# pkorus/neural-imaging

Measured on AMD Instinct MI355X. Metric: patches/s (fwd+bwd) ISP->JPEG->FAN @256^2, higher is better.
Workload: dtype bf16; 1 GPU; c4 = train_manipulation UNet->[native,sharpen:1,resample:50,gaussian:0.83,jpeg:80]->dJPEG(QF80,soft)->FAN, ds none, trainable nip+fan, lambda_nip 0.1; raw_patch=128, batch_per_gpu=64, global_batch=64, parallelism=dp1, world_size=1, hip_graph=False

## Files before the change

### include/nimg.h

```cpp
#ifndef NIMG_H
#define NIMG_H

#include <stddef.h>
#include <stdint.h>

#ifdef __cplusplus
extern "C" {
#endif

#define NIMG_OK 0
#define NIMG_ERR_ARG (-1)
#define NIMG_ERR_LAUNCH (-2)
#define NIMG_ERR_WORKSPACE (-3)

#define NIMG_BF16_IN 1
#define NIMG_BF16_OUT 2
#define NIMG_BF16_MASK 4
#define NIMG_BF16_DZ 8
#define NIMG_D2S_OUT 16
#define NIMG_MASK_CONV 128
#define NIMG_COPY_LRELU 64
#define NIMG_S2D_OUT 32
#define NIMG_UNPOOL_OUT 512
#define NIMG_D2S_CONVT 1024
// ... 232 lines not shown
int nimg_latent_fwd(const float* z, const float* scale, const float* codebook, int codebook_size, float v,
                    float gamma, int soft_codebook, float* latent, float* entropy, long count, long count_global,
                    void* workspace, size_t workspace_bytes, int finalize, void* stream);
int nimg_latent_entropy_finalize(int codebook_size, long count_global, float* entropy, void* workspace, void* stream);
int nimg_latent_bwd(const float* z, const float* scale, const float* latent, const float* dlatent,
                    float entropy_coef, const float* codebook, int codebook_size, float v, float gamma,
                    int soft_codebook, float* dz, float* dscale, int accumulate_dscale, long count, void* workspace,
                    size_t workspace_bytes, void* stream);
size_t nimg_l2_loss_workspace_bytes(void);
int nimg_l2_loss(const float* target, const float* y, float* loss, float* grad_y, long count, float grad_scale,
                 int accumulate, void* workspace, size_t workspace_bytes, void* stream);

size_t nimg_conv_weights_bf16_bytes(int ks_h, int ks_w, int cin, int cout, int mode);
int nimg_conv_weights_bf16(const float* w, void* wb, int ks_h, int ks_w, int cin, int cout, int mode, void* stream);
int nimg_conv2d_wgrad_pooled_bf16(const float* in, int cin, const float* g, const unsigned char* idx, int cout,
                                  float* dw, float* db, int n, int h, int wd, int ks, int accumulate, void* workspace,
                                  size_t workspace_bytes, void* stream);
int nimg_conv2d_dgrad_fewin_pooled_bf16(const float* g, const unsigned char* idx, const float* w, float* out, int ci,
                                        int cz, int n, int h, int wd, int ks, void* stream);
int nimg_conv2d_fwd_bf16_ex(const float* in1, int c1, const float* in2, int c2, const void* wb, const float* bias,
                            float* out1, int o1, float* out2, int o2, const float* act_mask, int n, int h, int wd,
                            int ks, int stride, int pad_t, int pad_l, int pad_mode, int hout, int wout, int act,
                            float alpha, int flags, void* stream);
int nimg_conv2d_wgrad_bf16_ex(const float* in1, int c1, const float* in2, int c2, const float* dz, int cout, float* dw,
                              float* db, int n, int h, int wd, int ks, int stride, int pad_t, int pad_l, int pad_mode,
                              int hout, int wout, int accumulate, void* workspace, size_t workspace_bytes, int flags,
                              void* stream);
int nimg_conv2d_pool_fwd_bf16_ex(const float* in, int cin, const float* w, const void* wb, const float* bias,
                                 float* pool_out, unsigned char* pool_idx, int cout, int n, int h, int wd, int ks,
                                 int act, float alpha, int flags, void* stream);
int nimg_conv2d_fwd_pool_also_bf16(const float* in, int cin, const void* wb, const float* bias, float* out, float* pool_out,
                                   unsigned char* pool_idx, int cout, int n, int h, int wd, int act, float alpha, void* stream);
#define NIMG_ROWS_F32_OUT 1
int nimg_conv3_rows_bf16(const void* in1, int c1, const void* in2, int c2, const void* wb, const float* bias, const void* mask,
                         void* out, void* out2, void* pool_out, int n, int h, int wd, int cout, int act, float alpha, int flags,
                         void* stream);
int nimg_conv3_rows_d2s_bf16(const void* in, int c1, const void* wb, const float* bias, float* y, int n, int h, int wd, void* stream);
int nimg_conv3_rows_c4_bf16(const float* in, const float* w, const float* bias, void* out, int n, int h, int wd, int act, float alpha,
                            void* stream);

int nimg_conv2d_dgrad_unpool_out_bf16(const float* dz, int c1, const void* wb, const float* act, const float* skip, float* out,
                                      int cout, int n, int h, int wd, int apply_mask, float alpha, void* stream);
int nimg_conv2d_wgrad_pooled_bf16_ex(const float* in, int cin, const float* g, const unsigned char* idx, int cout,
                                     float* dw, float* db, int n, int h, int wd, int ks, int accumulate, void* workspace,
                                     size_t workspace_bytes, int flags, void* stream);
int nimg_conv2d_dgrad_fewin_pooled_bf16_ex(const float* g, const unsigned char* idx, const float* w, float* out, int ci,
                                           int cz, int n, int h, int wd, int ks, int flags, void* stream);
int nimg_maxpool2_unpool_ex(const float* dp, const unsigned char* idx, const float* pooled, float* dz, int n, int ho,
                            int wo, int c, int apply_lrelu_mask, float alpha, int flags, void* stream);
int nimg_convt2x2_fwd_bf16(const float* x, const void* wb, const float* bias, float* y, int n, int h, int wd, int cin,
                           int cout, void* stream);
int nimg_convt2x2_fwd_bf16_ex(const float* x, const void* wb, const float* bias, float* y, int n, int h, int wd, int cin,
                              int cout, int flags, void* stream);
int nimg_conv_weights_bf16_batch(const void* table, int n_entries, void* stream);
int nimg_conv2d_fwd_bf16(const float* in1, int c1, const float* in2, int c2, const void* wb, const float* bias,
                         float* out1, int o1, float* out2, int o2, const float* act_mask, int n, int h, int wd,
                         int ks, int stride, int pad_t, int pad_l, int pad_mode, int hout, int wout, int act,
                         float alpha, void* stream);
size_t nimg_conv2d_wgrad_bf16_workspace_bytes(int cin, int cout, int ks_h, int ks_w, int n, int hout, int wout);
int nimg_conv2d_wgrad_bf16(const float* in1, int c1, const float* in2, int c2, const float* dz, int cout, float* dw,
                           float* db, int n, int h, int wd, int ks, int stride, int pad_t, int pad_l, int pad_mode,
                           int hout, int wout, int accumulate, void* workspace, size_t workspace_bytes, void* stream);

int nimg_conv2d_fwd_smallc_bf16(const float* in, int cin, const float* w, const float* bias, float* out, int cout,
                                int n, int h, int wd, int ks, int pad_mode, int act, float alpha, void* stream);
int nimg_conv2d_fwd_smallc_bf16_ex(const float* in, int cin, const float* w, const float* bias, float* out, int cout,
                                   int n, int h, int wd, int ks, int pad_mode, int act, float alpha, int flags, void* stream);
int nimg_conv2d_dgrad_fewin_bf16(const float* dz, const float* w, float* out, int ci, int cz, int n, int h, int wd,
                                 int ks, void* stream);

int nimg_awgn_fwd(const float* x, const float* noise, float* y, uint8_t* mask, long count, float strength,
                  void* stream);
int nimg_awgn_bwd(const float* x, const float* noise, const float* dy, const uint8_t* mask, float* dx, long count,
                  float strength, void* stream);
int nimg_gamma_fwd(const float* x, float* y, long count, float gamma, void* stream);
int nimg_gamma_bwd(const float* x, const float* dy, float* dx, long count, float gamma, void* stream);
int nimg_median_fwd(const float* x, float* y, uint8_t* sel, int n, int h, int w, int kernel, void* stream);
int nimg_median_bwd(const float* dy, const uint8_t* sel, float* dx, int n, int h, int w, int kernel, void* stream);

#define NIMG_L3IC_E_READ 1
#define NIMG_L3IC_E_LANES 2
#define NIMG_L3IC_E_RANGE 4
#define NIMG_L3IC_E_SYMBOL 8
#define NIMG_L3IC_E_FREQ 16
#define NIMG_L3IC_E_VARINT 32
#define NIMG_L3IC_E_ODD 64
#define NIMG_L3IC_E_UNUSED 128
#define NIMG_L3IC_E_STATE 256
#define NIMG_L3IC_E_RLE 512
size_t nimg_l3ic_workspace_bytes(int n_streams, int n_sym);
int nimg_l3ic_quantise(const float* z, const float* codebook, int codebook_size, uint8_t* idx, int* err, int n, int h,
                       int w, int c, void* stream);
int nimg_l3ic_encode(const uint8_t* idx, int n_streams, int n_sym, uint8_t* out, uint32_t* lengths, uint32_t* hist,
                     uint32_t* freq, void* workspace, size_t workspace_bytes, void* stream);
int nimg_l3ic_decode(const uint8_t* data, const uint32_t* offsets, const uint32_t* lengths, const float* codebook,
                     int codebook_size, float* z, uint32_t* err, int n, int h, int w, int c, void* stream);

size_t nimg_jpeg_workspace_bytes(int n, int h, int w, int hs, int vs);
int nimg_jpeg_transform(const void* x, int is_u8, int n, int h, int w, int hs, int vs, int quality, int16_t* coef, void* workspace,
                        size_t workspace_bytes, void* stream);
int nimg_jpeg_encode(const int16_t* coef, int n, int h, int w, int hs, int vs, uint8_t* out, size_t out_capacity, uint32_t* lengths,
                     void* workspace, size_t workspace_bytes, void* stream);
int nimg_jpeg_reconstruct(const int16_t* coef, int n, int h, int w, int hs, int vs, int quality, float* y, void* workspace,
                          size_t workspace_bytes, void* stream);
int nimg_jpeg_transform_items(const void* x, int is_u8, int n_src, int h, int w, int hs, int vs, const uint8_t* quality, int n_items,
                              int16_t* coef, int* err, void* workspace, size_t workspace_bytes, void* stream);
// ... 65 lines not shown
```

### neural-imaging_amd/_lib.py

```python
import ctypes
import os
from ctypes import c_float, c_int, c_long, c_size_t, c_void_p

_HERE = os.path.dirname(os.path.abspath(__file__))
LIB_PATH = os.environ.get('NIMG_LIBPATH') or os.path.join(_HERE, 'libnimg.so')

P = c_void_p

PROTOTYPES = {
    'nimg_abi_version': (c_int, []),
    'nimg_djpeg_fwd': (c_int, [P, P, P, P, P, P, c_int, c_int, c_int, c_int, P]),
    'nimg_djpeg_bwd': (c_int, [P, P, P, P, P, c_int, c_int, c_int, c_int, P]),
    'nimg_djpeg_dq_workspace_bytes': (c_size_t, [c_int, c_int, c_int]),
    'nimg_djpeg_bwd_dq': (c_int, [P, P, P, P, P, P, c_int, c_int, c_int, c_int, c_int, P, c_size_t, P]),
    'nimg_djpeg_sub_workspace_bytes': (c_size_t, [c_int, c_int, c_int, c_int, c_int, c_int]),
    'nimg_djpeg_sub_fwd': (c_int, [P, P, P, P, P, P, c_int, c_int, c_int, c_int, c_int, c_int, P, c_size_t, P]),
    'nimg_djpeg_sub_bwd': (c_int, [P, P, P, P, P, P, c_int, c_int, c_int, c_int, c_int, c_int, c_int, P, c_size_t, P]),
    'nimg_djpeg_entropy_workspace_bytes': (c_size_t, [c_int, c_int, c_int]),
    'nimg_djpeg_entropy_fwd': (c_int, [P, P, c_int, c_int, c_int, c_int, P, P, c_size_t, P]),
    'nimg_djpeg_entropy_bwd': (c_int, [P, P, c_int, c_int, c_int, c_int, c_float, P, c_int, P, c_int, P, c_size_t, P]),
    'nimg_jpeg_qtable': (c_int, [c_int, c_int, P]),
    'nimg_conv2d_fwd': (c_int, [P, c_int, P, c_int, P, P, P, c_int, P, c_int, P, c_int, c_int, c_int, c_int, c_int,
                                c_int, c_int, c_int, c_int, c_int, c_int, c_float, P]),
    'nimg_conv_flip_weights': (c_int, [P, P, c_int, c_int, c_int, c_int, P]),
# ... 94 lines not shown
    'nimg_isp_residual_workspace_bytes': (c_long, []),
    'nimg_isp_residual_bwd': (c_int, [P, P, P, P, P, P, c_long, c_int, P]),
    'nimg_activation_fwd': (c_int, [P, P, c_long, c_int, c_float, P]),
    'nimg_activation_bwd': (c_int, [P, P, P, c_long, c_int, c_float, P]),
    'nimg_sigmoid_fwd': (c_int, [P, P, c_long, P]),
    'nimg_sigmoid_bwd': (c_int, [P, P, P, c_long, P]),
    'nimg_gamma_ste_fwd': (c_int, [P, P, c_long, c_float, c_float, c_float, P]),
    'nimg_gamma_ste_bwd': (c_int, [P, P, P, c_long, c_float, c_float, c_float, P]),
    'nimg_mae255_workspace_bytes': (c_size_t, []),
    'nimg_mae255': (c_int, [P, P, P, P, c_long, c_float, c_int, P, c_size_t, P]),
    'nimg_ssim_loss_workspace_bytes': (c_size_t, [c_int, c_int, c_int, c_int, c_int]),
    'nimg_ssim_loss': (c_int, [P, P, P, P, c_int, c_int, c_int, c_int, c_float, P, c_float, c_int, P, c_size_t, P]),
    'nimg_patch_stats': (c_int, [P, c_int, c_int, c_int, P, P, c_int, c_int, c_int, P, P, P]),
    'nimg_patch_select': (c_int, [P, P, P, P, c_int, c_int, c_int, c_int, P, P, P]),
    'nimg_patch_gather': (c_int, [P, P, c_int, c_int, c_int, P, P, c_int, c_int, P, P, P]),
    'nimg_mask_scale': (c_int, [P, P, P, c_long, c_float, P]),
    'nimg_conv5_dgrad_sparse_image_bytes': (c_size_t, [c_int, c_int]),
    'nimg_conv5_dgrad_sparse_weights': (c_int, [P, P, c_int, c_int, P]),
    'nimg_conv5_dgrad_sparse': (c_int, [P, P, c_int, P, P, c_int, P, c_int, c_int, c_int, c_float, c_int, P]),
    'nimg_conv2d_fwd_bf16_res': (c_int, [P, c_int, P, P, P, c_int, P, P, P, c_int, c_int, c_int, c_int, c_int, c_int, c_int, c_int, c_int,
                                 c_int, c_int, c_float, c_int, P]),
    'nimg_conv2d_fwd_bf16_unpool': (c_int, [P, P, c_int, P, P, P, c_int, P, c_int, c_int, c_int, c_int, c_int, c_int, c_int,
                                            c_int, c_int, c_float, c_int, P]),
    'nimg_conv2d_wgrad_bf16_unpool': (c_int, [P, c_int, P, P, c_int, P, P, c_int, c_int, c_int, c_int, c_int, P, c_size_t, P]),
    'nimg_cconv3': (c_int, [P, P, P, P, c_int, c_int, c_int, c_int, P]),
    'nimg_conv5c3_bf16': (c_int, [P, P, P, c_int, c_int, c_int, P]),
    'nimg_cconv3_dgrad_border': (c_int, [P, P, P, c_int, c_int, c_int, P]),
    'nimg_cconv3_dgrad_border_strips': (c_int, [P, P, P, c_int, c_int, c_int, P]),
    'nimg_conv1_pool_fwd_c4': (c_int, [P, P, P, P, P, c_int, c_int, c_int, c_float, c_int, P]),
    'nimg_conv1_wgrad_c4_workspace_bytes': (c_size_t, []),
    'nimg_conv1_wgrad_c4': (c_int, [P, P, P, P, P, c_int, c_int, c_int, c_int, c_int, P, c_size_t, P]),
    'nimg_conv1_dgrad_pooled': (c_int, [P, P, P, P, c_int, c_int, c_int, c_int, P]),
    'nimg_confusion_accumulate': (c_int, [P, P, P, P, c_int, c_int, P]),
    'nimg_ssim_planes_workspace_bytes': (c_size_t, [c_int, c_int]),
    'nimg_ssim_planes': (c_int, [P, P, c_int, c_int, c_int, c_int, c_float, P, P, P, P, c_int, P, c_size_t, P]),
    'nimg_msssim_combine': (c_int, [P, P, c_int, c_int, P, P, P]),
    'nimg_ssim_maps_grad': (c_int, [P, P, P, P, P, c_int, c_int, c_int, c_int, P, c_float, c_int, P]),
    'nimg_pad2d': (c_int, [P, P, c_int, c_int, c_int, c_int, c_int, c_int, P]),
    'nimg_conv2d_fwd_bf16_ex': (c_int, [P, c_int, P, c_int, P, P, P, c_int, P, c_int, P, c_int, c_int, c_int, c_int, c_int,
                                        c_int, c_int, c_int, c_int, c_int, c_int, c_float, c_int, P]),
    'nimg_conv2d_wgrad_bf16_ex': (c_int, [P, c_int, P, c_int, P, c_int, P, P, c_int, c_int, c_int, c_int, c_int, c_int,
                                          c_int, c_int, c_int, c_int, c_int, P, c_size_t, c_int, P]),
    'nimg_conv2d_pool_fwd_bf16_ex': (c_int, [P, c_int, P, P, P, P, P, c_int, c_int, c_int, c_int, c_int, c_int, c_float,
                                             c_int, P]),
    'nimg_conv2d_dgrad_unpool_out_bf16': (c_int, [P, c_int, P, P, P, P, c_int, c_int, c_int, c_int, c_int, c_float, P]),
    'nimg_conv2d_fwd_pool_also_bf16': (c_int, [P, c_int, P, P, P, P, P, c_int, c_int, c_int, c_int, c_int, c_float, P]),
    'nimg_conv2d_wgrad_pooled_bf16_ex': (c_int, [P, c_int, P, P, c_int, P, P, c_int, c_int, c_int, c_int, c_int, P,
                                                 c_size_t, c_int, P]),
    'nimg_conv2d_dgrad_fewin_pooled_bf16_ex': (c_int, [P, P, P, P, c_int, c_int, c_int, c_int, c_int, c_int, c_int, P]),
    'nimg_maxpool2_unpool_ex': (c_int, [P, P, P, P, c_int, c_int, c_int, c_int, c_int, c_float, c_int, P]),
    'nimg_conv_weights_bf16_batch': (c_int, [P, c_int, P]),
    'nimg_convt2x2_fwd_bf16': (c_int, [P, P, P, P, c_int, c_int, c_int, c_int, c_int, P]),
    'nimg_convt2x2_fwd_bf16_ex': (c_int, [P, P, P, P, c_int, c_int, c_int, c_int, c_int, c_int, P]),
    'nimg_conv2d_fwd_smallc_bf16': (c_int, [P, c_int, P, P, P, c_int, c_int, c_int, c_int, c_int, c_int, c_int,
                                            c_float, P]),
    'nimg_conv2d_fwd_smallc_bf16_ex': (c_int, [P, c_int, P, P, P, c_int, c_int, c_int, c_int, c_int, c_int, c_int,
                                               c_float, c_int, P]),
    'nimg_conv2d_dgrad_fewin_bf16': (c_int, [P, P, P, c_int, c_int, c_int, c_int, c_int, c_int, P]),
    'nimg_awgn_fwd': (c_int, [P, P, P, P, c_long, c_float, P]),
    'nimg_awgn_bwd': (c_int, [P, P, P, P, P, c_long, c_float, P]),
    'nimg_gamma_fwd': (c_int, [P, P, c_long, c_float, P]),
    'nimg_gamma_bwd': (c_int, [P, P, P, c_long, c_float, P]),
    'nimg_median_fwd': (c_int, [P, P, P, c_int, c_int, c_int, c_int, P]),
    'nimg_median_bwd': (c_int, [P, P, P, c_int, c_int, c_int, c_int, P]),
    'nimg_sparse_axis_apply': (c_int, [P, P, P, P, P, c_int, c_int, c_int, c_int, c_int, c_int, P]),
    'nimg_l3ic_workspace_bytes': (c_size_t, [c_int, c_int]),
    'nimg_l3ic_quantise': (c_int, [P, P, c_int, P, P, c_int, c_int, c_int, c_int, P]),
    'nimg_l3ic_encode': (c_int, [P, c_int, c_int, P, P, P, P, P, c_size_t, P]),
    'nimg_l3ic_decode': (c_int, [P, P, P, P, c_int, P, P, c_int, c_int, c_int, c_int, P]),
    'nimg_jpeg_workspace_bytes': (c_size_t, [c_int, c_int, c_int, c_int, c_int]),
    'nimg_jpeg_transform': (c_int, [P, c_int, c_int, c_int, c_int, c_int, c_int, c_int, P, P, c_size_t, P]),
    'nimg_jpeg_encode': (c_int, [P, c_int, c_int, c_int, c_int, c_int, P, c_size_t, P, P, c_size_t, P]),
    'nimg_jpeg_reconstruct': (c_int, [P, c_int, c_int, c_int, c_int, c_int, c_int, P, P, c_size_t, P]),
    'nimg_jpeg_transform_items': (c_int, [P, c_int, c_int, c_int, c_int, c_int, c_int, P, c_int, P, P, P, c_size_t, P]),
    'nimg_jpeg_reconstruct_items': (c_int, [P, c_int, c_int, c_int, c_int, c_int, P, P, P, P, c_size_t, P]),
    'nimg_jpeg_decode_workspace_bytes': (c_size_t, [c_int, c_int, c_int, c_int, c_int, c_size_t, c_int]),
    'nimg_jpeg_decode': (c_int, [P, P, P, c_int, c_int, c_int, c_int, c_int, c_int, P, P, P, P, c_size_t, P]),
    'nimg_jpeg_reconstruct_tables': (c_int, [P, c_int, c_int, c_int, c_int, c_int, P, P, c_int, P, c_size_t, P]),
    'nimg_jpeg_histogram': (c_int, [P, c_int, c_int, c_int, c_int, c_int, P, P]),
    'nimg_jpeg_optimal_tables': (c_int, [P, c_int, P, P, P]),
    'nimg_jpeg_encode_tables_workspace_bytes': (c_size_t, [c_int, c_int, c_int, c_int, c_int]),
    'nimg_jpeg_encode_tables': (c_int, [P, c_int, c_int, c_int, c_int, c_int, P, P, c_size_t, P, P, P, c_size_t, P]),
    'nimg_jpeg_transform_tables': (c_int, [P, c_int, c_int, c_int, c_int, c_int, c_int, P, c_int, P, P, P, c_size_t, P]),
    'nimg_jpeg_tables_from_float': (c_int, [P, c_int, c_int, P, P, P]),
    'nimg_jpeg_encode_restart_workspace_bytes': (c_size_t, [c_int, c_int, c_int, c_int, c_int, c_int]),
    'nimg_jpeg_encode_restart': (c_int, [P, c_int, c_int, c_int, c_int, c_int, c_int, P, c_size_t, P, P, c_size_t, P]),
    'nimg_jpeg_histogram_restart': (c_int, [P, c_int, c_int, c_int, c_int, c_int, c_int, P, P]),
    'nimg_jpeg_encode_tables_restart_workspace_bytes': (c_size_t, [c_int, c_int, c_int, c_int, c_int, c_int]),
    'nimg_jpeg_encode_tables_restart': (c_int, [P, c_int, c_int, c_int, c_int, c_int, c_int, P, P, c_size_t, P, P, P, c_size_t, P]),
    'nimg_jpeg_decode_restart_workspace_bytes': (c_size_t, [c_int, c_int, c_int, c_int, c_int, c_int, c_size_t, c_int]),
    'nimg_jpeg_decode_restart': (c_int, [P, P, P, c_int, c_int, c_int, c_int, c_int, c_int, c_int, P, P, P, P, c_size_t, P]),
    'nimg_jpeg_decode_progressive_workspace_bytes': (c_size_t, [c_int, c_int, c_int, c_int, c_int, c_int, c_int, c_size_t, c_int]),
    'nimg_jpeg_decode_progressive': (c_int, [P, P, P, c_int, P, c_int, c_int, c_int, c_int, c_int, c_int, c_int, P, P, P, P, c_size_t, P]),
    'nimg_jpeg_progressive_workspace_bytes': (c_size_t, [c_int, c_int, c_int, c_int, c_int, c_int]),
    'nimg_jpeg_progressive_histogram': (c_int, [P, c_int, c_int, c_int, c_int, c_int, c_int, P, P]),
    'nimg_jpeg_encode_progressive': (c_int, [P, c_int, c_int, c_int, c_int, c_int, c_int, P, P, c_size_t, P, P, P, c_size_t, P]),
    'nimg_msssim_workspace_bytes': (c_size_t, [c_int, c_int, c_int, c_int]),
    'nimg_msssim': (c_int, [P, P, c_int, c_int, c_int, c_int, c_float, P, P, P, c_size_t, P]),
    'nimg_conv1_pool_fwd_c4_sign': (c_int, [P, P, P, P, P, P, c_int, c_int, c_int, c_float, c_int, P]),
    'nimg_conv2d_pool_sign_ok': (c_int, [c_int, c_int, c_int, c_int, c_int, c_int, c_int]),
    'nimg_conv2d_pool_fwd_bf16_sign': (c_int, [P, c_int, P, P, P, P, P, P, c_int, c_int, c_int, c_int, c_int, c_int, c_float,
                                               c_int, P]),
    'nimg_conv2d_fwd_bf16_unpool_sign': (c_int, [P, P, c_int, P, P, P, c_int, P, P, c_int, c_int, c_int, c_int, c_int, c_int, c_int,
                                                 c_int, c_int, c_float, c_int, P]),
}

# ... 37 lines not shown
```

### neural-imaging_amd/models/layers.py

```python
import numpy as np
import torch

from .. import ops
from ..helpers import kernels as hk


FUSED_ACTIVATIONS = (None, 'leaky_relu')


def act_forward(y, activation):
    if isinstance(y, tuple):
        raise RuntimeError('a bf16 copy cannot be combined with activation {}'.format(activation))
    return ops.activation(y, activation, out=y)


class Conv2D(object):

    def __init__(self, name, ks, cin, cout, activation=None, stride=1, cin2=0, mask_activation='leaky_relu'):
        self.name, self.ks, self.cin, self.cin2, self.cout = name, ks, cin, cin2, cout
        self.activation, self.stride = activation, stride
        self.mask_activation = mask_activation

    def specs(self):
        return [(self.name + '/kernel', (self.ks, self.ks, self.cin + self.cin2, self.cout)),
# ... 72 lines not shown
        return ops.conv2d_dgrad(dz, store.p[self.name + '/kernel'], in_hw, stride=self.stride, act_mask=act_mask,
                                out=out, out2=out2, out_bf16=out_bf16, residual=residual, bf16_copy=bf16_copy,
                                s2d_out=s2d_out)


class Conv5x5Stride2Image(Conv2D):

    def s2d_ok(self, x):
        return ops.s2d_conv_ok(self.ks, self.stride, x.shape[1], x.shape[2], self.cin) and self.cin2 == 0 and 4 * self.cin <= 16

    def forward_image(self, store, x, a, b, s2d_out=False):
        if not self.s2d_ok(x):
            if s2d_out:
                raise RuntimeError('s2d_out needs the space-to-depth form of the layer')
            x0 = ops.affine(x, a, b)
            return self.forward(store, x0), x0
        xs = ops.s2d2_affine(x, a, b, cp=16)
        w3 = ops.s2d_conv_weights(store.p[self.name + '/kernel'], cp=16)
        fused = self.activation in FUSED_ACTIVATIONS
        y = ops.conv2d(xs, w3, store.p[self.name + '/bias'], act=self.activation if fused else None, s2d_out=s2d_out,
                       out_bf16=s2d_out)
        return (y if fused else act_forward(y, self.activation)), xs

    def backward_params_image(self, store, ctx, dz):
        if ctx.dtype != torch.bfloat16:
            return self.backward_params(store, ctx, dz)
        with ops.side_stream(ctx, dz, key=store.g[self.name + '/kernel'].data_ptr()):
            dw3 = ops.conv2d_wgrad(ctx, dz, 3, db=store.g[self.name + '/bias'])
            ops.s2d_conv_weights_bwd(dw3, store.g[self.name + '/kernel'])

    def backward_input_image(self, store, dz, in_hw, a):
        return ops.conv2d_dgrad_strided2(dz, store.p[self.name + '/kernel'], in_hw, scale=a)


class Conv2DTranspose2x2(object):

    def __init__(self, name, cin, cout):
        self.name, self.cin, self.cout = name, cin, cout

    def specs(self):
        return [(self.name + '/kernel', (2, 2, self.cout, self.cin)), (self.name + '/bias', (self.cout,))]

    def init(self, store, gen):
        from .tfmodel import glorot_uniform_
        k = torch.empty((2, 2, self.cout, self.cin), dtype=torch.float32)
        glorot_uniform_(k, self.cin * 4, self.cout * 4, gen)
        store.p[self.name + '/kernel'].copy_(k)
        store.p[self.name + '/bias'].zero_()

    def forward(self, store, x, out_bf16=False):
        return ops.convt2x2(x, store.p[self.name + '/kernel'], store.p[self.name + '/bias'], out_bf16=out_bf16)

    def backward_params(self, store, x, dy):
        ops.convt2x2_wgrad(x, dy, dw=store.g[self.name + '/kernel'], side=True)
        ops.bias_grad(dy, db=store.g[self.name + '/bias'], side=True)

    def backward_input(self, store, dy, act_mask=None, out_bf16=False, mask_activation='leaky_relu'):
        if act_mask is not None and mask_activation not in FUSED_ACTIVATIONS:
            d = ops.convt2x2_dgrad(dy, store.p[self.name + '/kernel'])
            return ops.activation_bwd(d, act_mask, mask_activation, out=d)
        return ops.convt2x2_dgrad(dy, store.p[self.name + '/kernel'], act_mask=act_mask, out_bf16=out_bf16)


class ConstrainedConv2D(object):

    def __init__(self, name='constrained', filter_strength=100.0):
        self.name, self.strength = name, float(filter_strength)

    def specs(self):
        return [(self.name + '/kernel', (5, 5, 3, 3))]

    def init(self, store, gen=None):
        store.p[self.name + '/kernel'].copy_(torch.from_numpy(hk.residual_init_filter().astype(np.float32)))
        if hasattr(store, 'register_constrained'):
            store.register_constrained(self.name + '/kernel', self.strength)

    _flip = (None, None)

    def forward(self, store, x, c4_only=False):
        cc = getattr(store, 'constrained', None)
        if ops.ADAM_IMAGES and ops.ADAM_CCONV and ops.COMPUTE == 'bf16' and cc is not None and \
                cc['kernel'] is store.p[self.name + '/kernel'] and cc['strength'] == self.strength:
            nf, flip = store.constrained_filter()
            self._flip = (nf, flip)
        else:
            nf = ops.constrained_kernel(store.p[self.name + '/kernel'], self.strength)
            self._flip = (None, None)
        y, c4 = ops.cconv3(x, nf, pad_mode=1, want_f32=not c4_only, want_c4=c4_only)
        return (c4 if c4_only else y), nf

    def backward_params(self, store, x, dy):
        with ops.side_stream(x, dy, key=store.g[self.name + '/kernel'].data_ptr()):
            dnf = ops.conv2d_wgrad(x, dy, 5, pads=(2, 2), pad_mode=1)
            ops.constrained_kernel_bwd(store.p[self.name + '/kernel'], dnf, store.g[self.name + '/kernel'], self.strength)

    def backward_input(self, nf, dy):
        n, h, w, _ = dy.shape
        if h < 4 or w < 4:
            dpad = ops.conv2d(dy, ops.flip_weights(nf), None, pads=(4, 4), out_hw=(h + 4, w + 4))
            return ops.fold_pad(dpad, 2, 1)
        return ops.cconv3_dgrad(dy, nf, nf_flip=self._flip[1] if nf is self._flip[0] else None)
```

### neural-imaging_amd/ops.py

```python
import math
import os

import numpy as np
import torch

from . import _lib

LRELU_ALPHA = 0.2

COMPUTE = 'f32'


STORE_BF16 = True


COMPUTE_EPOCH = 0


def set_compute(mode):
    global COMPUTE, COMPUTE_EPOCH
    if mode not in ('f32', 'bf16'):
        raise ValueError('compute mode must be f32 or bf16')
    if mode != COMPUTE:
        COMPUTE_EPOCH += 1
# ... 778 lines not shown
        return dw
    if _is_bf16(x) or _is_bf16(dz):
        raise RuntimeError('bf16-stored tensor reached a float32 weight-gradient path')
    need = _lib.load().nimg_conv2d_wgrad_workspace_bytes(c1 + c2, cout, ks, ks, n, ho, wo)
    ws = _ws_current(x.device).get(need, x.device)
    _lib.call('nimg_conv2d_wgrad', _p(x), c1, _p(x2), c2, _p(dz), cout, _p(dw), _p(db), n, h, wd, ks, stride, pt, pl,
              pad_mode, ho, wo, 1 if accumulate else 0, _p(ws), ws.numel(), _stream())
    return dw


def _flush_chain_here(k):
    entry = _CHAIN.pop(k, None)
    if entry is not None:
        _lib.call('nimg_reduce_slabs_batch', entry, 1, _stream())


def _wgrad_carried(k, carrier, device, need, flags, *operands):
    import ctypes
    if carrier == 'defer':
        st = _defer_state(k)
        if st['n'] == st['cap']:
            _flush_deferred(k, on_its_stream=False)
        entry = ctypes.byref(st['buf'], st['n'] * st['nb'])
    else:
        entry = (ctypes.c_char * int(_lib.load().nimg_reduce_entry_bytes()))()
    ws = _SIDE['ws'][k].claim(need, device)
    name, pre = ('nimg_conv2d_wgrad_bf16_chained', (_CHAIN.get(k),)) if carrier == 'chain' else ('nimg_conv2d_wgrad_bf16_deferred', ())
    _lib.call(name, *operands, _p(ws), ws.numel(), flags, *pre, entry, _stream())
    if carrier == 'defer':
        st['n'] += 1
    elif carrier == 'chain':
        _CHAIN[k] = entry
    else:
        _reduce_behind(k, entry, device)


def bias_grad(dz, db=None, accumulate=False, side=False):
    if side and _SIDE['enabled'] and db is not None:
        with _on_side_stream(dz, key=db.data_ptr()):
            return bias_grad(dz, db=db, accumulate=accumulate, side=False)
    _f32(db)
    _fb(dz)
    cout = dz.shape[-1]
    npix = dz.numel() // cout
    if db is None:
        db = torch.empty((cout,), dtype=torch.float32, device=dz.device)
    need = _lib.load().nimg_bias_grad_workspace_bytes(npix, cout)
    ws = _ws_current(dz.device).get(need, dz.device)
    _lib.call('nimg_bias_grad_ex', _p(dz), _p(db), npix, cout, 1 if accumulate else 0, _p(ws), ws.numel(),
              BF16_DZ if _is_bf16(dz) else 0, _stream())
    return db


def convt2x2(x, w, bias, out_bf16=False):
    _f32(w, bias)
    _fb(x)
    n, h, wd, cin = x.shape
    cout = w.shape[2]
    y = torch.empty((n, 2 * h, 2 * wd, cout), dtype=torch.bfloat16 if out_bf16 else torch.float32, device=x.device)
    if COMPUTE == 'bf16' and cin % 8 == 0 and cout >= 8:
        wb = weights_bf16(w, 1)
        _lib.call('nimg_convt2x2_fwd_bf16_ex', _p(x), _p(wb), _p(bias), _p(y), n, h, wd, cin, cout,
                  (BF16_IN if _is_bf16(x) else 0) | (BF16_OUT if out_bf16 else 0), _stream())
        return y
    if _is_bf16(x) or out_bf16:
        raise RuntimeError('bf16-stored tensor reached a float32 transposed-convolution path')
    _lib.call('nimg_convt2x2_fwd', _p(x), _p(w), _p(bias), _p(y), n, h, wd, cin, cout, _stream())
    return y


def convt2x2_dgrad(dy, w, act_mask=None, out_bf16=False):
    n, h2, w2, _ = dy.shape
    return conv2d(dy, w, None, stride=2, pads=(0, 0), out_hw=(h2 // 2, w2 // 2), act_mask=act_mask, out_bf16=out_bf16)


def convt2x2_wgrad(x, dy, dw=None, side=False):
    return conv2d_wgrad(dy, x, 2, stride=2, pads=(0, 0), dw=dw, side=side)


def maxpool2(x):
    _fb(x)
    n, h, w, c = x.shape
    y = torch.empty((n, h // 2, w // 2, c), dtype=x.dtype, device=x.device)
    if _is_bf16(x):
        _lib.call('nimg_maxpool2_fwd_bf16', _p(x), _p(y), n, h, w, c, _stream())
        return y
    _lib.call('nimg_maxpool2_fwd', _p(x), _p(y), n, h, w, c, _stream())
    return y


def maxpool2_bwd(dp, yact, add=None, apply_mask=True, out=None, alpha=None):
    a = LRELU_ALPHA if alpha is None else float(alpha)
    _fb(dp, yact, add, out)
    n, h, w, c = yact.shape
    dz = torch.empty_like(yact) if out is None else out
    if _is_bf16(yact):
        if any(t is not None and not _is_bf16(t) for t in (dp, add, dz)):
            raise RuntimeError('maxpool2_bwd on a bf16-stored activation needs bf16-stored gradients')
        _lib.call('nimg_maxpool2_bwd_bf16', _p(dp), _p(yact), _p(add), _p(dz), n, h, w, c, 1 if apply_mask else 0,
                  a, _stream())
        return dz
    _f32(dp, add, dz)
    _lib.call('nimg_maxpool2_bwd', _p(dp), _p(yact), _p(add), _p(dz), n, h, w, c, 1 if apply_mask else 0,
              a, _stream())
    return dz


ACT_SIGN = _os.environ.get('NIMG_NO_ACT_SIGN') is None


def conv2d_pool_sign_ok(x, w, out_bf16=True):
    n, h, wd, cin = x.shape
    return ACT_SIGN and COMPUTE == 'bf16' and _is_bf16(x) and out_bf16 and _lib.load().nimg_conv2d_pool_sign_ok(
        cin, w.shape[3], n, h, wd, w.shape[0], BF16_IN | BF16_OUT) == 1


def conv2d_pool(x, w, bias=None, act='leaky_relu', want_idx=True, out_bf16=False, want_sign=False):
    _f32(w, bias)
    _fb(x)
    n, h, wd, cin = x.shape
    ks, cout = w.shape[0], w.shape[3]
    if w.shape[2] != cin or (h & 1) or (wd & 1) or (cout & 3) or ks not in (3, 5):
        raise ValueError('conv2d_pool: unsupported shape')
    bf16_path = COMPUTE == 'bf16' and (cin in (3, 4) or cin % 8 == 0)
    if (out_bf16 or _is_bf16(x)) and not bf16_path:
        raise RuntimeError('bf16 storage needs the throughput-mode convolution path')
    pooled = torch.empty((n, h // 2, wd // 2, cout), dtype=torch.bfloat16 if out_bf16 else torch.float32, device=x.device)
    idx = torch.empty((n, h // 2, wd // 2, cout), dtype=torch.uint8, device=x.device) if want_idx else None
    a = 1 if act == 'leaky_relu' else 0
    if bf16_path:
# ... 1537 lines not shown
```

Before: 8190 patches/s.

## Add dedicated MFMA GEMM kernels for transposed 2x2 conv fwd, dgrad and fused wgrad+bias

Result: no change. 8214 patches/s, median of 6 (+0.3%).

```diff
diff --git a/include/nimg.h b/include/nimg.h
--- a/include/nimg.h
+++ b/include/nimg.h
@@ -308,6 +308,14 @@
                            int cout, void* stream);
 int nimg_convt2x2_fwd_bf16_ex(const float* x, const void* wb, const float* bias, float* y, int n, int h, int wd, int cin,
                               int cout, int flags, void* stream);
+int nimg_convt2x2_gemm_ok(int pass, int n, int h, int wd, int cin, int cout, int flags);
+int nimg_convt2x2_gemm_fwd(const void* x, const void* wb, const float* bias, void* y, int n, int h, int wd, int cin, int cout,
+                           int flags, void* stream);
+int nimg_convt2x2_gemm_dgrad(const void* dy, const void* wb, const void* mask, void* dx, int n, int h, int wd, int cin, int cout,
+                             float alpha, int flags, void* stream);
+size_t nimg_convt2x2_gemm_wgrad_workspace_bytes(int n, int h, int wd, int cin, int cout);
+int nimg_convt2x2_gemm_wgrad_bias(const void* x, const void* dy, float* dw, float* db, int n, int h, int wd, int cin, int cout,
+                                  void* workspace, size_t workspace_bytes, int flags, void* stream);
 int nimg_conv_weights_bf16_batch(const void* table, int n_entries, void* stream);
 int nimg_conv2d_fwd_bf16(const float* in1, int c1, const float* in2, int c2, const void* wb, const float* bias,
                          float* out1, int o1, float* out2, int o2, const float* act_mask, int n, int h, int wd,
diff --git a/neural-imaging_amd/_lib.py b/neural-imaging_amd/_lib.py
--- a/neural-imaging_amd/_lib.py
+++ b/neural-imaging_amd/_lib.py
@@ -170,6 +170,11 @@
     'nimg_conv_weights_bf16_batch': (c_int, [P, c_int, P]),
     'nimg_convt2x2_fwd_bf16': (c_int, [P, P, P, P, c_int, c_int, c_int, c_int, c_int, P]),
     'nimg_convt2x2_fwd_bf16_ex': (c_int, [P, P, P, P, c_int, c_int, c_int, c_int, c_int, c_int, P]),
+    'nimg_convt2x2_gemm_ok': (c_int, [c_int, c_int, c_int, c_int, c_int, c_int, c_int]),
+    'nimg_convt2x2_gemm_fwd': (c_int, [P, P, P, P, c_int, c_int, c_int, c_int, c_int, c_int, P]),
+    'nimg_convt2x2_gemm_dgrad': (c_int, [P, P, P, P, c_int, c_int, c_int, c_int, c_int, c_float, c_int, P]),
+    'nimg_convt2x2_gemm_wgrad_workspace_bytes': (c_size_t, [c_int, c_int, c_int, c_int, c_int]),
+    'nimg_convt2x2_gemm_wgrad_bias': (c_int, [P, P, P, P, c_int, c_int, c_int, c_int, c_int, P, c_size_t, c_int, P]),
     'nimg_conv2d_fwd_smallc_bf16': (c_int, [P, c_int, P, P, P, c_int, c_int, c_int, c_int, c_int, c_int, c_int,
                                             c_float, P]),
     'nimg_conv2d_fwd_smallc_bf16_ex': (c_int, [P, c_int, P, P, P, c_int, c_int, c_int, c_int, c_int, c_int, c_int,
diff --git a/neural-imaging_amd/csrc/convt2x2.hip b/neural-imaging_amd/csrc/convt2x2.hip
--- /dev/null
+++ b/neural-imaging_amd/csrc/convt2x2.hip
@@ -0,0 +1,412 @@
+#include "conv_bf16_ring.h"
+
+namespace {
+
+constexpr int CG_TM = 128;
+constexpr int CG_A_ENT = CG_TM * 8;
+
+struct ConvtGemmParams {
+    const void* a;
+    const void* wb;
+    const float* bias;
+    const void* mask;
+    void* out;
+    int N, H, W;
+    int cin, cout;
+    int NC;
+    int stages;
+    float alpha;
+    int flags;
+    unsigned a_bytes, b_bytes;
+};
+
+template <int TN, int NS>
+size_t convt_gemm_lds(int stages) {
+    const size_t tiles = (size_t)(stages > 1 ? NS : 1) * (CG_A_ENT + TN * 8) * 16;
+    constexpr size_t epi = (size_t)4 * 32 * (TN / 2 + EPI_PAD) * sizeof(float);
+    return tiles > epi ? tiles : epi;
+}
+
+template <bool DGRAD, int TN, int NS>
+__global__ __launch_bounds__(256) void convt2x2_gemm_kernel(const ConvtGemmParams p) {
+    constexpr int MI = 2, NI = TN / 64, B_ENT = TN * 8;
+    constexpr int APW = CG_A_ENT / 64 / 4, BPW = B_ENT / 64 / 4;
+    extern __shared__ __attribute__((aligned(16))) unsigned char smem_raw[];
+    const int nbuf = p.stages > 1 ? NS : 1;
+    uint4* sA = reinterpret_cast<uint4*>(smem_raw);
+    uint4* sB = sA + nbuf * CG_A_ENT;
+    const unsigned lds0 = (unsigned)(unsigned long)(__attribute__((address_space(3))) unsigned char*)smem_raw;
+    const int tid = threadIdx.x, lane = tid & 63;
+    const int wave = __builtin_amdgcn_readfirstlane(tid >> 6);
+    const int wm = wave & 1, wn = wave >> 1, half = lane >> 5;
+    const int ct = p.NC / TN;
+    const int bid = xcd_order(blockIdx.x);
+    const int n0 = (bid % ct) * TN, m0 = (bid / ct) * CG_TM;
+    const int M = p.N * p.H * p.W;
+
+    unsigned aoff[APW], boff[BPW];
+#pragma unroll
+    for (int j = 0; j < APW; ++j) {
+        const int idx = (wave + 4 * j) * 64 + lane, row = idx >> 3, e = (idx & 7) ^ ((row >> 1) & 7);
+        const int pix = m0 + row, s = e >> 1, hf = e & 1;
+        unsigned off;
+        if constexpr (DGRAD) {
+            const int x = pix % p.W, y = (pix / p.W) % p.H, n = pix / (p.W * p.H);
+            const unsigned q = (unsigned)((n * 2 * p.H + 2 * y + (s >> 1)) * (2 * p.W) + 2 * x + (s & 1));
+            off = (q * (unsigned)p.cout + 8u * hf) * 2u;
+        } else {
+            off = ((unsigned)pix * (unsigned)p.cin + 16u * s + 8u * hf) * 2u;
+        }
+        aoff[j] = pix < M ? off : 0x80000000u;
+    }
+#pragma unroll
+    for (int j = 0; j < BPW; ++j) {
+        const int idx = (wave + 4 * j) * 64 + lane, row = idx >> 3, e = (idx & 7) ^ ((row >> 1) & 7);
+        boff[j] = (unsigned)((((e >> 1) * p.NC + n0 + row) * 16 + 8 * (e & 1)) * 2);
+    }
+    const unsigned long a_addr = (unsigned long)p.a, b_addr = (unsigned long)p.wb;
+    const r_u32x4 ra = {(unsigned)a_addr, (unsigned)(a_addr >> 32) & 0xffffu, p.a_bytes, 0x00020000u};
+    const r_u32x4 rb = {(unsigned)b_addr, (unsigned)(b_addr >> 32) & 0xffffu, p.b_bytes, 0x00020000u};
+    auto issue = [&](int st, int buf) {
+        const int sa = DGRAD ? st * 32 : st * 128, sb = st * 4 * p.NC * 32;
+#pragma unroll
+        for (int j = 0; j < APW; ++j)
+            glds16(ra, lds0 + (unsigned)((buf * CG_A_ENT + (wave + 4 * j) * 64) * 16), aoff[j], sa);
+#pragma unroll
+        for (int j = 0; j < BPW; ++j)
+            glds16(rb, lds0 + (unsigned)((nbuf * CG_A_ENT + buf * B_ENT + (wave + 4 * j) * 64) * 16), boff[j], sb);
+    };
+
+    f32x16 acc[MI][NI];
+#pragma unroll
+    for (int mi = 0; mi < MI; ++mi)
+#pragma unroll
+        for (int ni = 0; ni < NI; ++ni)
+#pragma unroll
+            for (int j = 0; j < 16; ++j) acc[mi][ni][j] = 0.0f;
+    int arow[MI], brow[NI];
+#pragma unroll
+    for (int mi = 0; mi < MI; ++mi) arow[mi] = (wm * MI + mi) * 32 + (lane & 31);
+#pragma unroll
+    for (int ni = 0; ni < NI; ++ni) brow[ni] = (wn * NI + ni) * 32 + (lane & 31);
+
+#pragma unroll
+    for (int s = 0; s < (NS > 2 ? NS - 1 : 1); ++s)
+        if (s < p.stages) issue(s, s);
+    dma_wait();
+    __syncthreads();
+    for (int st = 0, buf = 0, nxt = NS - 1; st < p.stages; ++st) {
+        const bool more = st + NS - 1 < p.stages;
+        if (more) issue(st + NS - 1, nxt);
+        const uint4* tA = sA + buf * CG_A_ENT;
+        const uint4* tB = sB + buf * B_ENT;
+#pragma unroll
+        for (int s = 0; s < 4; ++s) {
+            bf16x8 a[MI], b[NI];
+#pragma unroll
+            for (int mi = 0; mi < MI; ++mi) {
+                const uint4 v = tA[arow[mi] * 8 + ((2 * s + half) ^ ((arow[mi] >> 1) & 7))];
+                a[mi] = *reinterpret_cast<const bf16x8*>(&v);
+            }
+#pragma unroll
+            for (int ni = 0; ni < NI; ++ni) {
+                const uint4 v = tB[brow[ni] * 8 + ((2 * s + half) ^ ((brow[ni] >> 1) & 7))];
+                b[ni] = *reinterpret_cast<const bf16x8*>(&v);
+            }
+#pragma unroll
+            for (int mi = 0; mi < MI; ++mi)
+#pragma unroll
+                for (int ni = 0; ni < NI; ++ni)
+                    acc[mi][ni] = __builtin_amdgcn_mfma_f32_32x32x16_bf16(a[mi], b[ni], acc[mi][ni], 0, 0, 0);
+        }
+        if (more) dma_wait_leave<(NS - 2) * (APW + BPW)>();
+        else dma_wait();
+        asm volatile("s_waitcnt lgkmcnt(0)\n\ts_barrier" ::: "memory");
+        buf = buf + 1 == NS ? 0 : buf + 1;
+        nxt = nxt + 1 == NS ? 0 : nxt + 1;
+    }
+
+    float* elds = reinterpret_cast<float*>(smem_raw) + wave * (32 * (NI * 32 + EPI_PAD));
+    const int cbase = n0 + wn * NI * 32;
+    auto out_index = [&](int pix, int col) -> long {
+        if constexpr (DGRAD) return (long)pix * p.cin + col;
+        const int x = pix % p.W, y = (pix / p.W) % p.H, n = pix / (p.W * p.H);
+        const int blk = col / p.cout, ph = 3 - blk;
+        return (((long)n * 2 * p.H + 2 * y + (ph >> 1)) * (2 * p.W) + 2 * x + (ph & 1)) * p.cout + (col - blk * p.cout);
+    };
+#pragma unroll
+    for (int mi = 0; mi < MI; ++mi) {
+        const int pbase = m0 + (wm * MI + mi) * 32;
+        if (p.flags & NIMG_BF16_OUT) {
+            epilogue_via_lds8<NI>(acc[mi], elds, lane, [&](int row, int c, float4 lo, float4 hi) {
+                const int pix = pbase + row, col = cbase + c;
+                if (pix >= M) return;
+                const long o = out_index(pix, col);
+                float f[8] = {lo.x, lo.y, lo.z, lo.w, hi.x, hi.y, hi.z, hi.w};
+                if constexpr (DGRAD) {
+                    if (p.mask) {
+                        float m[8];
+                        if (p.flags & NIMG_BF16_MASK) {
+                            const bf16x8 mv = *reinterpret_cast<const bf16x8*>(reinterpret_cast<const __bf16*>(p.mask) + o);
+#pragma unroll
+                            for (int e = 0; e < 8; ++e) m[e] = (float)mv[e];
+                        } else {
+                            const float4 m0v = *reinterpret_cast<const float4*>(reinterpret_cast<const float*>(p.mask) + o);
+                            const float4 m1v = *reinterpret_cast<const float4*>(reinterpret_cast<const float*>(p.mask) + o + 4);
+                            m[0] = m0v.x; m[1] = m0v.y; m[2] = m0v.z; m[3] = m0v.w; m[4] = m1v.x; m[5] = m1v.y; m[6] = m1v.z; m[7] = m1v.w;
+                        }
+#pragma unroll
+                        for (int e = 0; e < 8; ++e) f[e] *= m[e] > 0.f ? 1.0f : p.alpha;
+                    }
+                } else if (p.bias) {
+                    const float* bp = p.bias + col % p.cout;
+                    const float4 b0 = *reinterpret_cast<const float4*>(bp), b1 = *reinterpret_cast<const float4*>(bp + 4);
+                    f[0] += b0.x; f[1] += b0.y; f[2] += b0.z; f[3] += b0.w; f[4] += b1.x; f[5] += b1.y; f[6] += b1.z; f[7] += b1.w;
+                }
+                *reinterpret_cast<bf16x8*>(reinterpret_cast<__bf16*>(p.out) + o) = pack8(f);
+            });
+        } else {
+            epilogue_via_lds<NI, false>(acc[mi], elds, lane, [&](int row, int c, float4 v) {
+                const int pix = pbase + row, col = cbase + c;
+                if (pix >= M) return;
+                const long o = out_index(pix, col);
+                if constexpr (DGRAD) {
+                    if (p.mask) {
+                        const float4 m = (p.flags & NIMG_BF16_MASK) ? load4_bf16(reinterpret_cast<const float*>(p.mask), o)
+                                                                     : *reinterpret_cast<const float4*>(reinterpret_cast<const float*>(p.mask) + o);
+                        v.x *= m.x > 0.f ? 1.0f : p.alpha; v.y *= m.y > 0.f ? 1.0f : p.alpha;
+                        v.z *= m.z > 0.f ? 1.0f : p.alpha; v.w *= m.w > 0.f ? 1.0f : p.alpha;
+                    }
+                } else if (p.bias) {
+                    const float4 b = *reinterpret_cast<const float4*>(p.bias + col % p.cout);
+                    v.x += b.x; v.y += b.y; v.z += b.z; v.w += b.w;
+                }
+                *reinterpret_cast<float4*>(reinterpret_cast<float*>(p.out) + o) = v;
+            });
+        }
+    }
+}
+
+template <bool DGRAD, int TN, int NS = 2>
+int launch_convt_gemm(const ConvtGemmParams& p, hipStream_t s) {
+    const long blocks = (long)(p.NC / TN) * cdiv(p.N * p.H * p.W, CG_TM);
+    if constexpr (NS == 2) {
+        if (p.stages >= 4 && blocks <= 256) return launch_convt_gemm<DGRAD, TN, 4>(p, s);
+    }
+    const size_t lds = convt_gemm_lds<TN, NS>(p.stages);
+    auto k = convt2x2_gemm_kernel<DGRAD, TN, NS>;
+    (void)hipFuncSetAttribute((const void*)k, hipFuncAttributeMaxDynamicSharedMemorySize, (int)convt_gemm_lds<TN, NS>(2));
+    hipLaunchKernelGGL(k, dim3((unsigned)blocks), dim3(256), lds, s, p);
+    NIMG_CHECK_LAUNCH();
+    return NIMG_OK;
+}
+
+typedef short cw_s16x4 __attribute__((ext_vector_type(4)));
+typedef short cw_s16x8 __attribute__((ext_vector_type(8)));
+__device__ __forceinline__ bf16x8 cw_tr_read8(const unsigned char* a0, const unsigned char* a1) {
+    const cw_s16x4 lo = __builtin_amdgcn_ds_read_tr16_b64_v4i16((cw_s16x4 __attribute__((address_space(3)))*)a0);
+    const cw_s16x4 hi = __builtin_amdgcn_ds_read_tr16_b64_v4i16((cw_s16x4 __attribute__((address_space(3)))*)a1);
+    cw_s16x8 r;
+    r[0] = lo[0]; r[1] = lo[1]; r[2] = lo[2]; r[3] = lo[3]; r[4] = hi[0]; r[5] = hi[1]; r[6] = hi[2]; r[7] = hi[3];
+    return *reinterpret_cast<bf16x8*>(&r);
+}
+
+constexpr int CW_KP = 64;
+constexpr int CW_Y_ENT = CW_KP * 16;
+
+struct ConvtWgradParams {
+    const void* x;
+    const void* dy;
+    float* partial;
+    float* db_partial;
+    int H, W, cin, cout, M;
+    int pps;
+    unsigned dy_bytes;
+};
+
+template <int TCI>
+__global__ __launch_bounds__(256) void convt2x2_wgrad_kernel(const ConvtWgradParams p) {
+    constexpr int NI = TCI / 32, XS = TCI / 8, X_ENT = CW_KP * XS;
+    constexpr int XPW = X_ENT / 64 / 4, YPW = CW_Y_ENT / 64 / 4;
+    extern __shared__ __attribute__((aligned(16))) unsigned char smem_raw[];
+    const unsigned lds0 = (unsigned)(unsigned long)(__attribute__((address_space(3))) unsigned char*)smem_raw;
+    const int tid = threadIdx.x, lane = tid & 63;
+    const int wave = __builtin_amdgcn_readfirstlane(tid >> 6);
+    const int half = lane >> 5, g = lane & 15, sub = (lane >> 4) & 1;
+    const int cit = p.cin / TCI, cot = p.cout / 32;
+    int bid = xcd_order(blockIdx.x);
+    const int ci0 = (bid % cit) * TCI;
+    bid /= cit;
+    const int co0 = (bid % cot) * 32, split = bid / cot;
+    const int kb = split * p.pps, kend = min(p.M, kb + p.pps);
+    const int stages = (kend - kb + CW_KP - 1) / CW_KP;
+    const bool do_bias = p.db_partial != nullptr && ci0 == 0;
+
+    const unsigned long x_addr = (unsigned long)p.x, y_addr = (unsigned long)p.dy;
+    const r_u32x4 rx = {(unsigned)x_addr, (unsigned)(x_addr >> 32) & 0xffffu, (unsigned)p.M * (unsigned)p.cin * 2u, 0x00020000u};
+    const r_u32x4 ry = {(unsigned)y_addr, (unsigned)(y_addr >> 32) & 0xffffu, p.dy_bytes, 0x00020000u};
+    unsigned xoff[XPW];
+#pragma unroll
+    for (int j = 0; j < XPW; ++j) {
+        const int L = (wave + 4 * j) * 64 + lane, row = L / XS, slot = (L % XS) ^ ((row & 3) << 1);
+        xoff[j] = ((unsigned)(kb + row) * (unsigned)p.cin + (unsigned)(ci0 + slot * 8)) * 2u;
+    }
+    auto issue = [&](int st, int buf) {
+#pragma unroll
+        for (int j = 0; j < XPW; ++j)
+            glds16(rx, lds0 + (unsigned)((buf * X_ENT + (wave + 4 * j) * 64) * 16),
+                   kb + st * CW_KP + ((wave + 4 * j) * 64 + lane) / XS < kend ? xoff[j] : 0x80000000u, st * CW_KP * p.cin * 2);
+#pragma unroll
+        for (int j = 0; j < YPW; ++j) {
+            const int L = (wave + 4 * j) * 64 + lane, row = L >> 4, slot = (L & 15) ^ ((row & 3) << 1), tap = slot >> 2;
+            const unsigned px = (unsigned)(kb + st * CW_KP + row), r = px / (unsigned)p.W, xx = px - r * (unsigned)p.W;
+            const unsigned q = 4u * p.W * r + 2u * xx + (tap >> 1) * 2u * p.W + (tap & 1);
+            const unsigned off = (q * (unsigned)p.cout + (unsigned)(co0 + (slot & 3) * 8)) * 2u;
+            glds16(ry, lds0 + (unsigned)((2 * X_ENT + buf * CW_Y_ENT + (wave + 4 * j) * 64) * 16), (int)px < kend ? off : 0x80000000u, 0);
+        }
+    };
+
+    f32x16 acc[NI], accb;
+#pragma unroll
+    for (int j = 0; j < 16; ++j) accb[j] = 0.0f;
+#pragma unroll
+    for (int ni = 0; ni < NI; ++ni)
+#pragma unroll
+        for (int j = 0; j < 16; ++j) acc[ni][j] = 0.0f;
+    bf16x8 ones;
+#pragma unroll
+    for (int e = 0; e < 8; ++e) ones[e] = (__bf16)1.0f;
+    const int sw = (g >> 2) << 1, rl = half * 8 + (g >> 2), inslot = (g & 1) * 8, slow = sub * 2 + ((g & 3) >> 1);
+    const unsigned ya = (unsigned)(rl * 256 + (((wave * 4 + slow) ^ sw) * 16) + inslot);
+    unsigned xa[NI];
+#pragma unroll
+    for (int ni = 0; ni < NI; ++ni) xa[ni] = (unsigned)(rl * XS * 16 + (((ni * 4 + slow) ^ sw) * 16) + inslot);
+
+    if (stages > 0) issue(0, 0);
+    dma_wait();
+    __syncthreads();
+    for (int st = 0, buf = 0; st < stages; ++st, buf ^= 1) {
+        if (st + 1 < stages) issue(st + 1, buf ^ 1);
+        const unsigned char* tX = smem_raw + buf * X_ENT * 16;
+        const unsigned char* tY = smem_raw + (2 * X_ENT + buf * CW_Y_ENT) * 16;
+#pragma unroll
+        for (int ks = 0; ks < CW_KP / 16; ++ks) {
+            const unsigned char* yr = tY + ks * 16 * 256 + ya;
+            const bf16x8 a = cw_tr_read8(yr, yr + 4 * 256);
+            bf16x8 b[NI];
+#pragma unroll
+            for (int ni = 0; ni < NI; ++ni) {
+                const unsigned char* xr = tX + ks * 16 * XS * 16 + xa[ni];
+                b[ni] = cw_tr_read8(xr, xr + 4 * XS * 16);
+            }
+#pragma unroll
+            for (int ni = 0; ni < NI; ++ni) acc[ni] = __builtin_amdgcn_mfma_f32_32x32x16_bf16(a, b[ni], acc[ni], 0, 0, 0);
+            if (do_bias) accb = __builtin_amdgcn_mfma_f32_32x32x16_bf16(a, ones, accb, 0, 0, 0);
+        }
+        dma_wait();
+        __syncthreads();
+    }
+    float* slab = p.partial + (long)split * 4 * p.cout * p.cin;
+#pragma unroll
+    for (int ni = 0; ni < NI; ++ni)
+#pragma unroll
+        for (int j = 0; j < 16; ++j) {
+            const int co = co0 + (j & 3) + 8 * (j >> 2) + 4 * half;
+            slab[((long)wave * p.cout + co) * p.cin + ci0 + ni * 32 + (lane & 31)] = acc[ni][j];
+        }
+    if (do_bias) {
+        float* red = reinterpret_cast<float*>(smem_raw);
+        if ((lane & 31) == 0) {
+#pragma unroll
+            for (int j = 0; j < 16; ++j) red[wave * 32 + (j & 3) + 8 * (j >> 2) + 4 * half] = accb[j];
+        }
+        __syncthreads();
+        if (tid < 32) p.db_partial[(long)split * p.cout + co0 + tid] = ((red[tid] + red[32 + tid]) + red[64 + tid]) + red[96 + tid];
+    }
+}
+
+struct ConvtWgradPlan { int splits, pps; };
+inline ConvtWgradPlan convt_wgrad_plan(long px, int cin, int cout) {
+    const long tiles = (long)(cout / 32) * (cin / (cin % 128 == 0 ? 128 : 64));
+    long splits = (512 + tiles - 1) / tiles;
+    const long most = (px + CW_KP - 1) / CW_KP;
+    if (splits > most) splits = most;
+    const long pps = ((px + splits - 1) / splits + CW_KP - 1) / CW_KP * CW_KP;
+    return ConvtWgradPlan{(int)((px + pps - 1) / pps), (int)pps};
+}
+
+constexpr long CG_MAX_BYTES = (1l << 31) - 65536;
+
+}
+
+extern "C" {
+
+int nimg_convt2x2_gemm_ok(int pass, int n, int h, int wd, int cin, int cout, int flags) {
+    if (n <= 0 || h <= 0 || wd <= 0 || cin <= 0 || cout <= 0) return 0;
+    if (!(flags & NIMG_BF16_IN)) return 0;
+    const long px = (long)n * h * wd;
+    if (px * cin * 4 >= CG_MAX_BYTES || px * 4 * cout * 4 >= CG_MAX_BYTES) return 0;
+    if (pass == 0) {
+        if (flags & ~(NIMG_BF16_IN | NIMG_BF16_OUT)) return 0;
+        return cin % 64 == 0 && cout % 32 == 0 && (cin == 64 || cin >= 256);
+    }
+    if (pass == 1) {
+        if (flags & ~(NIMG_BF16_IN | NIMG_BF16_OUT | NIMG_BF16_MASK)) return 0;
+        return cout % 16 == 0 && cin % 64 == 0;
+    }
+    if (pass == 2)
+        return flags == (NIMG_BF16_IN | NIMG_BF16_DZ) && cin % 64 == 0 && cout % 32 == 0;
+    return 0;
+}
+
+size_t nimg_convt2x2_gemm_wgrad_workspace_bytes(int n, int h, int wd, int cin, int cout) {
+    if (!nimg_convt2x2_gemm_ok(2, n, h, wd, cin, cout, NIMG_BF16_IN | NIMG_BF16_DZ)) return 0;
+    return (size_t)convt_wgrad_plan((long)n * h * wd, cin, cout).splits * ((size_t)4 * cout * cin + cout) * sizeof(float);
+}
+
+int nimg_convt2x2_gemm_wgrad_bias(const void* x, const void* dy, float* dw, float* db, int n, int h, int wd, int cin, int cout,
+                                  void* workspace, size_t workspace_bytes, int flags, void* stream) {
+    if (!x || !dy || !dw || !workspace || !nimg_convt2x2_gemm_ok(2, n, h, wd, cin, cout, flags)) return NIMG_ERR_ARG;
+    if (workspace_bytes < nimg_convt2x2_gemm_wgrad_workspace_bytes(n, h, wd, cin, cout)) return NIMG_ERR_WORKSPACE;
+    const long px = (long)n * h * wd;
+    const ConvtWgradPlan plan = convt_wgrad_plan(px, cin, cout);
+    const long count = (long)4 * cout * cin;
+    ConvtWgradParams p;
+    p.x = x; p.dy = dy; p.partial = (float*)workspace; p.db_partial = db ? p.partial + (size_t)plan.splits * count : nullptr;
+    p.H = h; p.W = wd; p.cin = cin; p.cout = cout; p.M = (int)px; p.pps = plan.pps; p.dy_bytes = (unsigned)(px * 4 * cout * 2);
+    hipStream_t s = (hipStream_t)stream;
+    const bool wide = cin % 128 == 0;
+    const long blocks = (long)(cout / 32) * (cin / (wide ? 128 : 64)) * plan.splits;
+    const size_t lds = (size_t)2 * (CW_KP * (wide ? 16 : 8) + CW_Y_ENT) * 16;
+    auto k = wide ? convt2x2_wgrad_kernel<128> : convt2x2_wgrad_kernel<64>;
+    (void)hipFuncSetAttribute((const void*)k, hipFuncAttributeMaxDynamicSharedMemorySize, (int)lds);
+    hipLaunchKernelGGL(k, dim3((unsigned)blocks), dim3(256), lds, s, p);
+    NIMG_CHECK_LAUNCH();
+    launch_reduce2(p.partial, dw, count, plan.splits, p.db_partial, db, (long)cout, plan.splits, 0, s);
+    NIMG_CHECK_LAUNCH();
+    return NIMG_OK;
+}
+
+int nimg_convt2x2_gemm_fwd(const void* x, const void* wb, const float* bias, void* y, int n, int h, int wd, int cin, int cout,
+                           int flags, void* stream) {
+    if (!x || !wb || !y || !nimg_convt2x2_gemm_ok(0, n, h, wd, cin, cout, flags)) return NIMG_ERR_ARG;
+    ConvtGemmParams p;
+    p.a = x; p.wb = wb; p.bias = bias; p.mask = nullptr; p.out = y; p.N = n; p.H = h; p.W = wd; p.cin = cin; p.cout = cout;
+    p.NC = 4 * cout; p.stages = cin / 64; p.alpha = 0.f; p.flags = flags;
+    p.a_bytes = (unsigned)((long)n * h * wd * cin * 2); p.b_bytes = (unsigned)((long)cin * cout * 8);
+    return launch_convt_gemm<false, 128>(p, (hipStream_t)stream);
+}
+
+int nimg_convt2x2_gemm_dgrad(const void* dy, const void* wb, const void* mask, void* dx, int n, int h, int wd, int cin, int cout,
+                             float alpha, int flags, void* stream) {
+    if (!dy || !wb || !dx || !nimg_convt2x2_gemm_ok(1, n, h, wd, cin, cout, flags)) return NIMG_ERR_ARG;
+    if ((flags & NIMG_BF16_MASK) && !mask) return NIMG_ERR_ARG;
+    ConvtGemmParams p;
+    p.a = dy; p.wb = wb; p.bias = nullptr; p.mask = mask; p.out = dx; p.N = n; p.H = h; p.W = wd; p.cin = cin; p.cout = cout;
+    p.NC = cin; p.stages = cout / 16; p.alpha = alpha; p.flags = flags;
+    p.a_bytes = (unsigned)((long)n * h * wd * 4 * cout * 2); p.b_bytes = (unsigned)((long)cin * cout * 8);
+    hipStream_t s = (hipStream_t)stream;
+    return cin % 128 == 0 ? launch_convt_gemm<true, 128>(p, s) : launch_convt_gemm<true, 64>(p, s);
+}
+
+}
diff --git a/neural-imaging_amd/models/layers.py b/neural-imaging_amd/models/layers.py
--- a/neural-imaging_amd/models/layers.py
+++ b/neural-imaging_amd/models/layers.py
@@ -148,6 +148,9 @@
         return ops.convt2x2(x, store.p[self.name + '/kernel'], store.p[self.name + '/bias'], out_bf16=out_bf16)
 
     def backward_params(self, store, x, dy):
+        if ops.convt2x2_wgrad_bias_ok(x, dy):
+            ops.convt2x2_wgrad_bias(x, dy, dw=store.g[self.name + '/kernel'], db=store.g[self.name + '/bias'], side=True)
+            return
         ops.convt2x2_wgrad(x, dy, dw=store.g[self.name + '/kernel'], side=True)
         ops.bias_grad(dy, db=store.g[self.name + '/bias'], side=True)
 
diff --git a/neural-imaging_amd/ops.py b/neural-imaging_amd/ops.py
--- a/neural-imaging_amd/ops.py
+++ b/neural-imaging_amd/ops.py
@@ -854,6 +854,13 @@
     return db
 
 
+CONVT_GEMM = _os.environ.get('NIMG_NO_CONVT_GEMM') is None
+
+
+def _convt_gemm_ok(pass_, n, h, wd, cin, cout, flags):
+    return CONVT_GEMM and COMPUTE == 'bf16' and bool(_lib.load().nimg_convt2x2_gemm_ok(pass_, n, h, wd, cin, cout, flags))
+
+
 def convt2x2(x, w, bias, out_bf16=False):
     _f32(w, bias)
     _fb(x)
@@ -862,8 +869,11 @@
     y = torch.empty((n, 2 * h, 2 * wd, cout), dtype=torch.bfloat16 if out_bf16 else torch.float32, device=x.device)
     if COMPUTE == 'bf16' and cin % 8 == 0 and cout >= 8:
         wb = weights_bf16(w, 1)
-        _lib.call('nimg_convt2x2_fwd_bf16_ex', _p(x), _p(wb), _p(bias), _p(y), n, h, wd, cin, cout,
-                  (BF16_IN if _is_bf16(x) else 0) | (BF16_OUT if out_bf16 else 0), _stream())
+        flags = (BF16_IN if _is_bf16(x) else 0) | (BF16_OUT if out_bf16 else 0)
+        if _convt_gemm_ok(0, n, h, wd, cin, cout, flags):
+            _lib.call('nimg_convt2x2_gemm_fwd', _p(x), _p(wb), _p(bias), _p(y), n, h, wd, cin, cout, flags, _stream())
+            return y
+        _lib.call('nimg_convt2x2_fwd_bf16_ex', _p(x), _p(wb), _p(bias), _p(y), n, h, wd, cin, cout, flags, _stream())
         return y
     if _is_bf16(x) or out_bf16:
         raise RuntimeError('bf16-stored tensor reached a float32 transposed-convolution path')
@@ -872,12 +882,49 @@
 
 
 def convt2x2_dgrad(dy, w, act_mask=None, out_bf16=False):
-    n, h2, w2, _ = dy.shape
+    n, h2, w2, cout = dy.shape
+    cin = w.shape[3]
+    flags = (BF16_IN if _is_bf16(dy) else 0) | (BF16_OUT if out_bf16 else 0) | (BF16_MASK if _is_bf16(act_mask) else 0)
+    if h2 % 2 == 0 and w2 % 2 == 0 and w.shape[2] == cout and \
+            (act_mask is None or tuple(act_mask.shape) == (n, h2 // 2, w2 // 2, cin)) and \
+            _convt_gemm_ok(1, n, h2 // 2, w2 // 2, cin, cout, flags):
+        _f32(w)
+        _fb(dy, act_mask)
+        dx = torch.empty((n, h2 // 2, w2 // 2, cin), dtype=torch.bfloat16 if out_bf16 else torch.float32, device=dy.device)
+        _lib.call('nimg_convt2x2_gemm_dgrad', _p(dy), _p(weights_bf16(w, 0)), _p(act_mask), _p(dx), n, h2 // 2, w2 // 2, cin, cout,
+                  LRELU_ALPHA, flags, _stream())
+        return dx
     return conv2d(dy, w, None, stride=2, pads=(0, 0), out_hw=(h2 // 2, w2 // 2), act_mask=act_mask, out_bf16=out_bf16)
 
 
 def convt2x2_wgrad(x, dy, dw=None, side=False):
     return conv2d_wgrad(dy, x, 2, stride=2, pads=(0, 0), dw=dw, side=side)
+
+
+def convt2x2_wgrad_bias_ok(x, dy):
+    n, h, wd, cin = x.shape
+    return tuple(dy.shape[:3]) == (n, 2 * h, 2 * wd) and \
+        _convt_gemm_ok(2, n, h, wd, cin, dy.shape[3], (BF16_IN if _is_bf16(x) else 0) | (BF16_DZ if _is_bf16(dy) else 0))
+
+
+def convt2x2_wgrad_bias(x, dy, dw=None, db=None, side=False):
+    if not convt2x2_wgrad_bias_ok(x, dy):
+        return convt2x2_wgrad(x, dy, dw=dw, side=side), bias_grad(dy, db=db, side=side)
+    if side and _SIDE['enabled'] and dw is not None and db is not None:
+        with _on_side_stream(x, dy, key=dw.data_ptr()):
+            return convt2x2_wgrad_bias(x, dy, dw=dw, db=db, side=False)
+    _f32(dw, db)
+    n, h, wd, cin = x.shape
+    cout = dy.shape[3]
+    if dw is None:
+        dw = torch.empty((2, 2, cout, cin), dtype=torch.float32, device=x.device)
+    if db is None:
+        db = torch.empty((cout,), dtype=torch.float32, device=x.device)
+    need = _lib.load().nimg_convt2x2_gemm_wgrad_workspace_bytes(n, h, wd, cin, cout)
+    ws = _ws_current(x.device).get(need, x.device)
+    _lib.call('nimg_convt2x2_gemm_wgrad_bias', _p(x), _p(dy), _p(dw), _p(db), n, h, wd, cin, cout, _p(ws), ws.numel(),
+              BF16_IN | BF16_DZ, _stream())
+    return dw, db
 
 
 def maxpool2(x):
```
